# kshedden/muscato

Hardware: AMD Instinct MI355X
Metric: reads/sec (100 bp, multi-map) at 1/2/4/8 MI355X; confirm-kernel HBM GB/s vs peak (higher is better)
Workload: dtype u32

## Files before the change

muscato_amd/build.py:

```python
from __future__ import annotations

import os
import shutil
import subprocess
from concurrent.futures import ThreadPoolExecutor

HERE = os.path.dirname(os.path.abspath(__file__))
CSRC = os.path.join(HERE, "csrc")
LIB = os.path.join(HERE, "libmuscato_hip.so")
OBJ = os.path.join(HERE, "build")
SOURCES = [os.path.join(CSRC, f) for f in ("muscato_hip.hip", "match_lane_rw4.hip", "match_lane_rw8.hip", "match_lane_rw12.hip",
                                           "match_lane_rw8w.hip", "match_lane_rw12w.hip", "match_lane_rw16w.hip", "match_lane_rw8s.hip", "match_dma_rw8.hip")]
HEADERS = [os.path.join(os.path.dirname(HERE), "include", "muscato_hip.h")] + \
    [os.path.join(CSRC, f) for f in sorted(os.listdir(CSRC)) if f.endswith(".hpp")]
LANE_ONLY = os.path.join(CSRC, "kernels_match_lane.hpp")
DMA_ONLY = os.path.join(CSRC, "kernels_match_dma.hpp")
FLAGS = ["--offload-arch=gfx950", "-O3", "-std=c++17", "-fPIC", "-Wall", "-Wno-unused-function"]


def hipcc() -> str:
    for cand in (shutil.which("hipcc"), "/opt/rocm/bin/hipcc"):
        if cand and os.path.exists(cand):
            return cand
    raise RuntimeError("hipcc not found: libmuscato_hip.so cannot be built")


def needs_build() -> bool:
    if not os.path.exists(LIB):
        return True
    t = os.path.getmtime(LIB)
    return any(os.path.getmtime(p) > t for p in SOURCES + HEADERS)


HOST = os.path.join(CSRC, "host")
BIN = os.path.join(HERE, "bin")
HOST_HEADERS = [os.path.join(HOST, f) for f in sorted(os.listdir(HOST)) if f.endswith(".hpp")]
TOOLS = {"muscato": "muscato_cli.cpp", "muscato_prep_targets": "muscato_prep_targets.cpp",
         "muscato_screen": "muscato_screen.cpp", "muscato_confirm": "muscato_confirm.cpp"}
GPU_TOOLS = ("muscato", "muscato_prep_targets", "muscato_screen", "muscato_confirm")


def build_tools(force: bool = False, verbose: bool = False) -> None:
    os.makedirs(BIN, exist_ok=True)
    for name, src in TOOLS.items():
        out = os.path.join(BIN, name)
        srcp = os.path.join(HOST, src)
        deps = [srcp] + HOST_HEADERS + HEADERS
        if not force and os.path.exists(out) and all(os.path.getmtime(d) <= os.path.getmtime(out) for d in deps):
            continue
        cmd = ["g++", "-O2", "-std=c++17", "-Wall", "-pthread", "-o", out, srcp, "-lz"]
        if name in GPU_TOOLS:
            cmd += ["-L" + HERE, "-lmuscato_hip", "-Wl,-rpath,$ORIGIN/.."]
        if verbose:
            print(" ".join(cmd))
        subprocess.check_call(cmd)


CHECKS = {"read_names_plan_check": ("read_names_plan_check.cpp", ("read_names_plan.hpp",))}
SANITIZE = ["-O1", "-g", "-fsanitize=address,undefined", "-fno-sanitize-recover=all", "-static-libasan", "-static-libubsan"]


def build_checks(force: bool = False, verbose: bool = False, sanitize: bool = False, out_dir: str = BIN) -> dict:
    os.makedirs(out_dir, exist_ok=True)
    built = {}
    for name, (src, hdrs) in CHECKS.items():
        out = os.path.join(out_dir, name + ("_san" if sanitize else ""))
        srcp = os.path.join(HOST, src)
        deps = [srcp] + [os.path.join(CSRC, h) for h in hdrs]
        if force or not os.path.exists(out) or any(os.path.getmtime(d) > os.path.getmtime(out) for d in deps):
            cmd = ["g++", "-std=c++17", "-Wall"] + (SANITIZE if sanitize else ["-O2"]) + ["-o", out, srcp]
            if verbose:
                print(" ".join(cmd))
            subprocess.check_call(cmd)
        built[name] = out
    return built


def _compile(src: str, force: bool, verbose: bool, defines=(), tag: str = "") -> str:
    obj = os.path.join(OBJ, os.path.basename(src) + tag + ".o")
    base = os.path.basename(src)
    deps = [src] + [h for h in HEADERS if (h != LANE_ONLY or "match_lane" in base or "match_dma" in base) and (h != DMA_ONLY or "match_dma" in base)]
    if not force and os.path.exists(obj) and all(os.path.getmtime(d) <= os.path.getmtime(obj) for d in deps):
        return obj
    cmd = [hipcc()] + FLAGS + list(defines) + ["-c", "-o", obj, src]
    if verbose:
        print(" ".join(cmd))
    subprocess.check_call(cmd)
    return obj


def build(force: bool = False, verbose: bool = False) -> str:
    if force or needs_build():
        os.makedirs(OBJ, exist_ok=True)
        with ThreadPoolExecutor(max_workers=len(SOURCES)) as ex:
            objs = list(ex.map(lambda s: _compile(s, force, verbose), SOURCES))
        cmd = [hipcc(), "--offload-arch=gfx950", "-shared", "-fPIC", "-o", LIB] + objs + ["-ldl"]
        if verbose:
            print(" ".join(cmd))
        subprocess.check_call(cmd)
    build_tools(force=force, verbose=verbose)
    build_checks(force=force, verbose=verbose)
    return LIB


def variant(name: str, defines) -> str:
    os.makedirs(OBJ, exist_ok=True)
    out_dir = os.path.join(os.path.dirname(HERE), "build_variants")
    os.makedirs(out_dir, exist_ok=True)
    with ThreadPoolExecutor(max_workers=len(SOURCES)) as ex:
        main_defs = ["-D" + d[len("-DMAIN_"):] for d in defines if d.startswith("-DMAIN_")]
        lane_defs = [d for d in defines if not d.startswith("-DMAIN_")]
        objs = list(ex.map(lambda s: _compile(s, False, False, lane_defs if ("match_lane" in s or "match_dma" in s) else main_defs,
                                              "." + name if (("match_lane" in s or "match_dma" in s) and lane_defs) or ("match_lane" not in s and "match_dma" not in s and main_defs) else ""), SOURCES))
    out = os.path.join(out_dir, name + ".so")
    subprocess.check_call([hipcc(), "--offload-arch=gfx950", "-shared", "-fPIC", "-o", out] + objs + ["-ldl"])
    return out


if __name__ == "__main__":
    import sys
    if len(sys.argv) > 2 and sys.argv[1] == "variant":
        print(variant(sys.argv[2], sys.argv[3:]))
    else:
        print(build(force="--force" in sys.argv, verbose=True))
```

muscato_amd/csrc/muscato_hip.hip:

```cpp

#include <hip/hip_runtime.h>
#include <rccl/rccl.h>
#include <dlfcn.h>

#include <algorithm>
#include <cstdarg>
#include <cstdio>
#include <cstdlib>
#include <cstring>
#include <map>
#include <mutex>
#include <string>
#include <type_traits>
#include <vector>

#include "../../include/muscato_hip.h"

#include "ctx_state.hpp"
#include "dev_mem.hpp"
#include "index_plan.hpp"
#include "load_plan.hpp"

#include "kernels_common.hpp"
#include "kernels_index.hpp"
// ... 56 lines not shown
    }
  }
};
const Roctx& roctx() {
  static const Roctx r;
  return r;
}
struct Range {
  bool on;
  explicit Range(const char* name) : on(roctx().push != nullptr) {
    if (on) (void)roctx().push(name);
  }
  ~Range() {
    if (on) (void)roctx().pop();
  }
};

struct CaptureGuard {
  hipStream_t st = nullptr;
  bool active = false;
  hipError_t begin(hipStream_t s) {
    const hipError_t e = hipStreamBeginCapture(s, hipStreamCaptureModeThreadLocal);
    if (e == hipSuccess) {
      st = s;
      active = true;
    }
    return e;
  }
  hipError_t end(hipGraph_t* g) {
    active = false;
    return hipStreamEndCapture(st, g);
  }
  ~CaptureGuard() {
    if (!active) return;
    hipGraph_t g = nullptr;
    (void)hipStreamEndCapture(st, &g);
    if (g) (void)hipGraphDestroy(g);
    (void)hipGetLastError();
  }
};

struct TmpBufs {
  void* p[16] = {};
  int n = 0;
  template <class T>
  hipError_t alloc(T** out, size_t bytes) {
    void* q = nullptr;
    *out = nullptr;
    if (n >= 16) return hipErrorOutOfMemory;
    const hipError_t e = hipMalloc(&q, bytes ? bytes : 16);
    if (e == hipSuccess) p[n++] = q;
    *out = (T*)q;
    return e;
  }
  void release() {
    for (int i = 0; i < n; i++) (void)hipFree(p[i]);
    n = 0;
  }
  ~TmpBufs() { release(); }
};

}

using musc_load::RecShape;
using musc_load::StreamPlan;
using musc_load::stream_plan;
using musc_load::stream_plan_batch;

struct EnvKnobs : musc_index::Knobs {
  bool match_dma = false;
  bool screen_wg = false;
  int context = 0;
  bool no_x_context = false;
  bool force_wide = false;
  int debug_grid = 0;
  bool debug_sync = false;
  int graph = -1;
  bool pipeline = false;
  bool no_spec = false;
  long batch_reads = 0;
  uint64_t stage_bytes = 64ull << 20;
  uint64_t stage_lines = 1ull << 20;
  long mm_heap_lds = 0;
  void read() {
    *this = EnvKnobs();
    auto is = [](const char* v, const char* w) { return v && !strcmp(v, w); };
    const char* e = getenv("MUSC_INDEX");
    index = is(e, "classic") ? musc_index::IDX_CLASSIC : is(e, "lines") ? musc_index::IDX_LINES : is(e, "classic64") ? musc_index::IDX_CLASSIC64 : musc_index::IDX_AUTO;
    e = getenv("MUSC_MATCH");
    match_dma = is(e, "dma");
    screen_wg = is(getenv("MUSC_SCREEN"), "wg");
    e = getenv("MUSC_CONTEXT");
    context = is(e, "narrow") ? 1 : is(e, "wide") ? 2 : 0;
    no_x_context = getenv("MUSC_NO_X_CONTEXT") != nullptr;
    force_wide = getenv("MUSC_DEBUG_FORCE_WIDE") != nullptr;
    if ((e = getenv("MUSC_DEBUG_INDEX_BITS"))) index_bits = atoi(e);
    ctx_direct = (e = getenv("MUSC_DEBUG_CTX_DIRECT")) && atoi(e) > 0;
    if ((e = getenv("MUSC_DEBUG_GRID"))) debug_grid = atoi(e);
    debug_sync = getenv("MUSC_DEBUG_SYNC") != nullptr;
    if ((e = getenv("MUSC_GRAPH"))) graph = atoi(e);
    if ((e = getenv("MUSC_PIPELINE"))) pipeline = atoi(e) > 0;
    no_spec = getenv("MUSC_NO_SPEC") != nullptr;
    if ((e = getenv("MUSC_BATCH_READS"))) batch_reads = atol(e);
    if ((e = getenv("MUSC_DEBUG_INDEX_BUDGET_MB"))) index_budget_mb = atol(e);
    if ((e = getenv("MUSC_DEBUG_STAGE_BYTES")) && atoll(e) > 0) stage_bytes = (uint64_t)atoll(e);
    if ((e = getenv("MUSC_DEBUG_STAGE_LINES")) && atoll(e) > 0) stage_lines = (uint64_t)atoll(e);
    if ((e = getenv("MUSC_DEBUG_MM_HEAP_LDS"))) mm_heap_lds = atol(e);
  }
};

struct musc_ctx {
  int device = 0;
  hipStream_t stream = nullptr;
  std::string err;
  EnvKnobs env;
  musc_state::State st;

  DevPtr<uint32_t> db2;
  DevPtr<uint32_t> dbm2;
  bool db_has_x = false;
  bool reads_have_x = false;
  DevBuf<uint32_t> rdx;
  struct { uint64_t gen = 0; int wide = -1; } rdx_of;
  struct { uint64_t gen = 0; double pmatch = -1.0; int32_t mmp1 = -1; bool ok = false; } xok;
  DevPtr<uint32_t> dbx;
  uint64_t max_tlen = 0;
  struct { uint64_t gen = 0; int32_t key[CTX_MAX_W + 3] = {0}; bool ok = false; } xokdb;
  DevPtr<uint64_t> seq_off;
  uint32_t nseq = 0;
  uint64_t nbases = 0;
  uint64_t db_words = 0;
  std::vector<uint64_t> h_seq_off;

  uint64_t part_bases = 0;
  std::vector<uint32_t> part_first;
  musc_index::Kind part_kind = musc_index::K_CLASSIC64;
  uint64_t part_size = 0;
  uint32_t cur_part = 0;
  DevBuf<musc_hit> pacc;
  DevBuf<uint32_t> pbest;
  DevBuf<uint64_t> pcnt, padj;
  DevBuf<uint32_t> pflags, pflags_tmp;
  DevBuf<uint32_t> block_acc;

  musc_index::Resident idx;
  int wide = 0;
  DevMem idx_T, idx_E, ctx_T, ctx_E;
  unsigned scrt_resident = 0;
  int scrt_rw = 0;
  uint64_t idx_novf = 0;
  DevPtr<PathParams> d_pp;
  PathParams h_pp;
  bool h_pp_valid = false;
  DevPtr<MatchParams> d_mp;
  MatchParams h_mp;
  bool h_mp_valid = false;
  int spec_geom = 0;
  DevBuf<uint4> spill;

  DevPtr<uint32_t> rd;
  uint64_t rd_cap = 0;
  DevPtr<uint32_t> rdm;
  uint64_t nreads = 0;
  int rw = 0;
  uint32_t max_len = 0;
  bool reads_failed = false;

  struct Upload {
    DevPtr<uint32_t> stage;
    hipStream_t s_up = nullptr;
    std::vector<hipEvent_t> ev;
    StreamPlan plan;
    uint64_t next_piece = 0;
    uint64_t packed_upto = 0;
    uint32_t L = 0;
    bool active = false;
  } up;

  struct BatchSet {
    DevBuf<uint32_t> wb, rvalid, tbase, tcount;
    DevBuf<uint4> cdesc;
  } bs[2];
  int cur = 0;
  hipStream_t stream2 = nullptr;
  hipStream_t s_confirm = nullptr;
  hipEvent_t ev_ready[2] = {nullptr, nullptr}, ev_free[2] = {nullptr, nullptr}, ev_join = nullptr;
  DevBuf<uint32_t> scan_tmp, tcount2, tpre;
  DevBuf<uint4> stage;
  DevBuf<uint32_t> p_nx;
  DevBuf<uint16_t> nmiss_tab;
// ... 1005 lines not shown
```

muscato_amd/csrc/muscato_prep.hpp:

```cpp

#include <rocprim/device/device_radix_sort.hpp>

#define PREP_BASES_PER_WORD 21

DEV uint32_t prep_code(unsigned char ch) {
  switch (ch) {
    case 'A': return 1u;
    case 'C': return 2u;
    case 'G': return 3u;
    case 'T': return 4u;
    default: return 5u;
  }
}

MUSC_KERNEL __launch_bounds__(256) void k_prep_keys(const unsigned char* __restrict__ s,
                                                   const uint64_t* __restrict__ off,
                                                   const uint32_t* __restrict__ perm, uint64_t n, uint32_t w,
                                                   uint64_t* __restrict__ keys) {
  for (uint64_t i = (uint64_t)blockIdx.x * blockDim.x + threadIdx.x; i < n; i += (uint64_t)gridDim.x * blockDim.x) {
    const uint32_t r = perm[i];
    const uint64_t o = off[r];
    const uint64_t len = off[r + 1] - o;
    const uint64_t first = (uint64_t)w * PREP_BASES_PER_WORD;
    uint64_t key = 0;
    for (uint32_t j = 0; j < PREP_BASES_PER_WORD; j++) {
      const uint64_t q = first + j;
      if (q >= len) break;
      key |= (uint64_t)prep_code(s[o + q]) << (60 - 3 * j);
    }
    keys[i] = key;
  }
}

MUSC_KERNEL void k_prep_iota(uint32_t* __restrict__ p, uint64_t n) {
  for (uint64_t i = (uint64_t)blockIdx.x * blockDim.x + threadIdx.x; i < n; i += (uint64_t)gridDim.x * blockDim.x)
    p[i] = (uint32_t)i;
}

MUSC_KERNEL __launch_bounds__(256) void k_prep_heads(const unsigned char* __restrict__ s,
                                                    const uint64_t* __restrict__ off,
                                                    const uint32_t* __restrict__ perm, uint64_t n,
                                                    uint32_t* __restrict__ head) {
  for (uint64_t i = (uint64_t)blockIdx.x * blockDim.x + threadIdx.x; i < n; i += (uint64_t)gridDim.x * blockDim.x) {
    uint32_t h = 1;
    if (i > 0) {
      const uint32_t a = perm[i], b = perm[i - 1];
      const uint64_t oa = off[a], ob = off[b];
      const uint64_t la = off[a + 1] - oa, lb = off[b + 1] - ob;
      if (la == lb) {
        h = 0;
        for (uint64_t q = 0; q < la; q++)
          if (s[oa + q] != s[ob + q]) {
            h = 1;
            break;
          }
      }
    }
    head[i] = h;
  }
}

MUSC_KERNEL void k_prep_starts(const uint32_t* __restrict__ head, const uint32_t* __restrict__ incl, uint64_t n,
                              uint32_t* __restrict__ ustart, uint32_t* __restrict__ uhead,
                              const uint32_t* __restrict__ perm) {
  for (uint64_t i = (uint64_t)blockIdx.x * blockDim.x + threadIdx.x; i < n; i += (uint64_t)gridDim.x * blockDim.x) {
    if (head[i]) {
      ustart[incl[i] - 1] = (uint32_t)i;
      uhead[incl[i] - 1] = perm[i];
    }
    if (i == n - 1) ustart[incl[i]] = (uint32_t)n;
  }
}

MUSC_KERNEL void k_prep_pack(const unsigned char* __restrict__ s, const uint64_t* __restrict__ off,
                            const uint32_t* __restrict__ uhead, uint64_t nunique, int rw,
                            uint32_t* __restrict__ rd, uint32_t* __restrict__ rdm, uint32_t* __restrict__ has_x) {
  const uint64_t t = (uint64_t)blockIdx.x * blockDim.x + threadIdx.x;
  const uint64_t g = t / rw;
  const int j = (int)(t % rw);
  if (g >= nunique) return;
  const uint32_t r = uhead[g];
  const uint64_t o = off[r];
  const uint32_t len = (uint32_t)(off[r + 1] - o);
  if (j == rw - 1) {
    uint32_t anyx = 0;
    for (uint32_t q = 0; q < len; q++) {
      uint32_t isx;
      (void)ascii_code(s[o + q], &isx);
      anyx |= isx;
    }
    rd[t] = (len & 0xFFFFu) | (anyx ? READ_HAS_X : 0u);
    rdm[t] = 0;
    return;
  }
  uint32_t v = 0, mv = 0;
  for (int b = 0; b < 16; b++) {
    const uint32_t q = (uint32_t)j * 16 + b;
    if (q < len) {
      uint32_t isx;
      const uint32_t c = ascii_code(s[o + q], &isx);
      v |= c << (2 * b);
      mv |= isx << (2 * b);
    }
  }
  rd[t] = v;
  rdm[t] = mv;
  if (mv) atomicOr(has_x, 1u);
}

static int reads_sort_unique_dev(musc_ctx* c, const char* who, const unsigned char* d_s, const uint64_t* d_off, const uint64_t n,
                                 const Marks& m, uint32_t** order, uint32_t** ustart, uint64_t* nunique) {
  TmpBufs B;
  RecShape shape;
  uint64_t first = 0, last = 0, maxlen = 0;
  int rc = offsets_census(c, d_off, n, &first, &last, &maxlen);
  if (rc) return rc;
  if (first != 0) return fail(c, 2, "read offsets[0] must be 0");
  if ((rc = reads_shape(c, 0, maxlen, false, &shape))) return rc;

  const uint32_t nw = (uint32_t)std::max<uint64_t>((maxlen + PREP_BASES_PER_WORD - 1) / PREP_BASES_PER_WORD, 1);
  uint64_t *k0 = nullptr, *k1 = nullptr;
  uint32_t *p0 = nullptr, *p1 = nullptr;
  if ((rc = tmp_alloc(c, who, B, &k0, n * 8)) || (rc = tmp_alloc(c, who, B, &k1, n * 8)) || (rc = tmp_alloc(c, who, B, &p0, n * 4)) ||
      (rc = tmp_alloc(c, who, B, &p1, n * 4)))
    return rc;
  size_t tmp_bytes = 0;
  HIPCHK(c, rocprim::radix_sort_pairs(nullptr, tmp_bytes, k0, k1, p0, p1, (size_t)n, 0u, 63u, c->stream));
  void* tmp = nullptr;
  if ((rc = tmp_alloc(c, who, B, &tmp, tmp_bytes))) return rc;
  const dim3 grid(std::min(nblk(n, 256), MAX_GRID));
  hipLaunchKernelGGL(k_prep_iota, grid, dim3(256), 0, c->stream, p0, n);
  HIPCHK(c, hipGetLastError());
  for (uint32_t w = nw; w-- > 0;) {
    hipLaunchKernelGGL(k_prep_keys, grid, dim3(256), 0, c->stream, d_s, d_off, p0, n, w, k0);
    HIPCHK(c, hipGetLastError());
    HIPCHK(c, rocprim::radix_sort_pairs(tmp, tmp_bytes, k0, k1, p0, p1, (size_t)n, 0u, 63u, c->stream));
    std::swap(p0, p1);
  }

  uint32_t *head = nullptr, *incl = nullptr, *stmp = nullptr, *d_ustart = nullptr, *d_uhead = nullptr;
  if ((rc = tmp_alloc(c, who, B, &head, n * 4)) || (rc = tmp_alloc(c, who, B, &incl, n * 4)) ||
      (rc = tmp_alloc(c, who, B, &stmp, scan_tmp_elems(n) * 4)) || (rc = tmp_alloc(c, who, B, &d_ustart, (n + 1) * 4)) ||
      (rc = tmp_alloc(c, who, B, &d_uhead, n * 4)))
    return rc;
  hipLaunchKernelGGL(k_prep_heads, grid, dim3(256), 0, c->stream, d_s, d_off, p0, n, head);
  HIPCHK(c, hipGetLastError());
  if ((rc = scan_u32(c, head, incl, n, true, stmp))) return rc;
  hipLaunchKernelGGL(k_prep_starts, grid, dim3(256), 0, c->stream, head, incl, n, d_ustart, d_uhead, p0);
  HIPCHK(c, hipGetLastError());
  uint32_t nu32 = 0;
  HIPCHK(c, hipMemcpyAsync(&nu32, incl + (n - 1), 4, hipMemcpyDeviceToHost, c->stream));
  HIPCHK(c, hipStreamSynchronize(c->stream));
  const uint64_t nu = nu32;

  if ((rc = reads_shape(c, nu, maxlen, false, &shape)) || (rc = reads_records(c, shape, nu, maxlen, true, false))) return rc;
  const auto [rw, words] = shape;
  uint32_t* d_hasx = c->d_flag;
  HIPCHK(c, hipMemsetAsync(d_hasx, 0, 4, c->stream));
  hipLaunchKernelGGL(k_prep_pack, dim3(nblk(words, 256)), dim3(256), 0, c->stream, d_s, d_off, d_uhead, nu, rw, c->rd,
                     c->rdm, d_hasx);
  HIPCHK(c, hipGetLastError());
  HIPCHK(c, m.mark(c, 1));

  uint32_t* h_order = (uint32_t*)malloc(n * 4);
  uint32_t* h_ustart = (uint32_t*)malloc((nu + 1) * 4);
  if (!h_order || !h_ustart) {
    free(h_order);
    free(h_ustart);
    return fail(c, 7, "out of host memory for the sort order");
  }
  uint32_t hasx = 0;
  hipError_t e = hipMemcpyAsync(h_order, p0, n * 4, hipMemcpyDeviceToHost, c->stream);
  if (e == hipSuccess) e = hipMemcpyAsync(h_ustart, d_ustart, (nu + 1) * 4, hipMemcpyDeviceToHost, c->stream);
  if (e == hipSuccess) e = hipMemcpyAsync(&hasx, d_hasx, 4, hipMemcpyDeviceToHost, c->stream);
  if (e == hipSuccess) e = hipStreamSynchronize(c->stream);
  if (e != hipSuccess) {
    free(h_order);
    free(h_ustart);
    return fail(c, 10, "musc_reads_sort_unique: %s", hipGetErrorString(e));
  }
  reads_settle_x(c, hasx);
  c->stats.ms_read_prep = m.ms(0, 1);
  *order = h_order;
  *ustart = h_ustart;
  *nunique = nu;
  return 0;
}

static int reads_sort_unique_run(musc_ctx* c, const char* seqs, const uint64_t* offsets, uint64_t nreads, int on_device,
                                 uint32_t** order, uint32_t** ustart, uint64_t* nunique) {
  HIPCHK(c, hipSetDevice(c->device));
  free_reads(c);
  if (nreads >= 0xFFFFFFF0ull) return fail(c, 2, "too many reads for 32-bit read numbers");
  if (nreads == 0) {
    c->rw = 4;
    *order = (uint32_t*)malloc(4);
    *ustart = (uint32_t*)calloc(1, 4);
    if (!*order || !*ustart) return fail(c, 7, "out of host memory");
    return 0;
  }
  static const char* const who = "musc_reads_sort_unique";
  Marks m;
  int rc = m.start(c);
  if (rc) return rc;
  TmpBufs B;
  const unsigned char* d_s = nullptr;
  const uint64_t* d_off = nullptr;
  if ((rc = staged(c, who, B, (const unsigned char*)seqs, on_device ? 0 : offsets[nreads], on_device, 64, &d_s)) ||
      (rc = staged(c, who, B, offsets, (nreads + 1) * 8, on_device, 0, &d_off)))
    return rc;
  HIPCHK(c, m.mark(c, 0));
  return reads_sort_unique_dev(c, who, d_s, d_off, nreads, m, order, ustart, nunique);
}

extern "C" int musc_reads_sort_unique(musc_ctx* c, const char* seqs, const uint64_t* offsets, uint64_t nreads,
                                      int on_device, uint32_t** order, uint32_t** ustart, uint64_t* nunique) {
  if (!c) return 1;
  if (!order || !ustart || !nunique) return fail(c, 2, "musc_reads_sort_unique: NULL output pointer");
  *order = *ustart = nullptr;
  *nunique = 0;
  if ((!seqs || !offsets) && nreads) return fail(c, 2, "musc_reads_sort_unique: NULL input");
  return reads_load_done(c, reads_sort_unique_run(c, seqs, offsets, nreads, on_device, order, ustart, nunique));
}


extern "C" void musc_fastq_prep_free(musc_fastq_prep* p) {
  if (!p) return;
  free(p->name_off);
// ... 103 lines not shown
```

Measured before the change: 2.092 billion.

## Sort reads by first key word then refine only tied runs

Replaces the full LSD radix sort over every key word of every read with a sort on the first 21-base word, followed by detection of tied runs. Only the reads in tied runs are re-sorted on the remaining words and then by segment, and the result is scattered back. This avoids a radix pass over all n reads for each extra word when most prefixes are unique. The cost is extra scans, gathers and kernels, and more complex correctness, which is covered by a new host-side checker. The old path is kept behind MUSC_PREP_SORT=lsd.

Result: no change. 2.092 billion (median of 4 runs) (-0.0%).

```diff
diff --git a/muscato_amd/build.py b/muscato_amd/build.py
--- a/muscato_amd/build.py
+++ b/muscato_amd/build.py
@@ -56,7 +56,8 @@
         subprocess.check_call(cmd)
 
 
-CHECKS = {"read_names_plan_check": ("read_names_plan_check.cpp", ("read_names_plan.hpp",))}
+CHECKS = {"read_names_plan_check": ("read_names_plan_check.cpp", ("read_names_plan.hpp",)),
+          "prep_sort_plan_check": ("prep_sort_plan_check.cpp", ("prep_sort_plan.hpp",))}
 SANITIZE = ["-O1", "-g", "-fsanitize=address,undefined", "-fno-sanitize-recover=all", "-static-libasan", "-static-libubsan"]
 
 
diff --git a/muscato_amd/csrc/host/prep_sort_plan_check.cpp b/muscato_amd/csrc/host/prep_sort_plan_check.cpp
--- /dev/null
+++ b/muscato_amd/csrc/host/prep_sort_plan_check.cpp
@@ -0,0 +1,250 @@
+#include <algorithm>
+#include <cstdio>
+#include <cstdlib>
+#include <numeric>
+#include <random>
+#include <string>
+#include <vector>
+
+#include "../prep_sort_plan.hpp"
+
+using namespace musc_ps;
+
+static long g_checks = 0;
+#define CHECK(cond, ...)                                       \
+  do {                                                         \
+    g_checks++;                                                \
+    if (!(cond)) {                                             \
+      fprintf(stderr, "FAILED %s:%d: %s -- ", __FILE__, __LINE__, #cond); \
+      fprintf(stderr, __VA_ARGS__);                            \
+      fprintf(stderr, "\n");                                   \
+      exit(1);                                                 \
+    }                                                          \
+  } while (0)
+
+typedef std::vector<std::string> Reads;
+
+static int rank_of(char ch) { return ch == 'A' ? 0 : ch == 'C' ? 1 : ch == 'G' ? 2 : ch == 'T' ? 3 : 4; }
+static bool seq_less(const std::string& a, const std::string& b) {
+  const size_t k = std::min(a.size(), b.size());
+  for (size_t i = 0; i < k; i++)
+    if (rank_of(a[i]) != rank_of(b[i])) return rank_of(a[i]) < rank_of(b[i]);
+  return a.size() < b.size();
+}
+
+static uint64_t key_word(const std::string& s, uint32_t w) {
+  uint64_t key = 0;
+  for (uint32_t j = 0; j < BASES_PER_WORD; j++) {
+    const uint64_t q = (uint64_t)w * BASES_PER_WORD + j;
+    if (q >= s.size()) break;
+    key |= (uint64_t)(rank_of(s[q]) + 1) << base_shift(j);
+  }
+  return key;
+}
+static uint64_t seen(uint64_t key, BitRange r) { return (key >> r.begin) & ((1ull << (r.end - r.begin)) - 1); }
+
+struct Result {
+  std::vector<uint32_t> order, head;
+  uint32_t nw = 0;
+  uint64_t m = 0, runs = 0;
+};
+
+static Result stage(const Reads& reads) {
+  Result R;
+  const uint64_t n = reads.size();
+  uint64_t maxlen = 0;
+  for (const std::string& s : reads) maxlen = std::max<uint64_t>(maxlen, s.size());
+  const uint32_t nw = R.nw = word_count(maxlen);
+  std::vector<uint32_t> p(n);
+  std::iota(p.begin(), p.end(), 0u);
+  const BitRange b0 = word_bits(maxlen, 0);
+  std::stable_sort(p.begin(), p.end(), [&](uint32_t a, uint32_t b) { return seen(key_word(reads[a], 0), b0) < seen(key_word(reads[b], 0), b0); });
+  std::vector<uint64_t> K0(n);
+  for (uint64_t i = 0; i < n; i++) K0[i] = key_word(reads[p[i]], 0);
+  std::vector<uint32_t> h0(n), r(n), tincl(n);
+  for (uint64_t i = 0; i < n; i++) h0[i] = run_head(K0.data(), i) ? 1u : 0u;
+  uint32_t acc = 0, tacc = 0;
+  for (uint64_t i = 0; i < n; i++) {
+    r[i] = acc += h0[i];
+    tincl[i] = tacc += tied(h0.data(), n, i) ? 1u : 0u;
+  }
+  const uint64_t runs = R.runs = acc, m = R.m = tacc;
+  if (nw > 1 && m > 0) {
+    std::vector<uint32_t> pos(m), q(m), seg(m);
+    for (uint64_t i = 0; i < n; i++)
+      if (tied(h0.data(), n, i)) {
+        const uint32_t k = tincl[i] - 1;
+        pos[k] = (uint32_t)i, q[k] = p[i], seg[k] = r[i] - 1;
+      }
+    std::vector<uint32_t> slot(m);
+    std::iota(slot.begin(), slot.end(), 0u);
+    for (uint32_t w = nw; w-- > 1;) {
+      const BitRange br = word_bits(maxlen, w);
+      std::stable_sort(slot.begin(), slot.end(),
+                       [&](uint32_t a, uint32_t b) { return seen(key_word(reads[q[a]], w), br) < seen(key_word(reads[q[b]], w), br); });
+    }
+    const uint32_t sbits = seg_bits(runs);
+    if (sbits) {
+      const BitRange br{0u, sbits};
+      std::stable_sort(slot.begin(), slot.end(), [&](uint32_t a, uint32_t b) { return seen(seg[a], br) < seen(seg[b], br); });
+    }
+    for (uint64_t k = 0; k < m; k++) p[pos[k]] = q[slot[k]];
+  }
+  R.head.resize(n);
+  for (uint64_t i = 0; i < n; i++) R.head[i] = (i == 0 || h0[i] || reads[p[i]] != reads[p[i - 1]]) ? 1u : 0u;
+  R.order = p;
+  return R;
+}
+
+static Result check_case(const char* name, const Reads& reads) {
+  const Result R = stage(reads);
+  const uint64_t n = reads.size();
+  std::vector<uint32_t> exp(n);
+  std::iota(exp.begin(), exp.end(), 0u);
+  std::stable_sort(exp.begin(), exp.end(), [&](uint32_t a, uint32_t b) { return seq_less(reads[a], reads[b]); });
+  CHECK(R.order.size() == n, "%s", name);
+  for (uint64_t i = 0; i < n; i++) {
+    CHECK(R.order[i] == exp[i], "%s: position %llu holds read %u, the reference has %u", name, (unsigned long long)i, R.order[i], exp[i]);
+    const uint32_t h = (i == 0 || reads[exp[i]] != reads[exp[i - 1]]) ? 1u : 0u;
+    CHECK(R.head[i] == h, "%s: head flag of position %llu", name, (unsigned long long)i);
+  }
+  return R;
+}
+
+static std::string rnd(std::mt19937& g, size_t len, const char* alphabet, size_t na) {
+  std::string s(len, 'A');
+  for (char& ch : s) ch = alphabet[g() % na];
+  return s;
+}
+static std::string differ_at(const std::string& s, size_t at) {
+  std::string t = s;
+  t[at] = t[at] == 'G' ? 'T' : 'G';
+  return t;
+}
+
+int main() {
+  for (uint64_t L = 0; L <= 5000; L++) {
+    const uint32_t nw = word_count(L);
+    CHECK(nw >= 1 && (uint64_t)nw * BASES_PER_WORD >= L && (nw == 1 || (uint64_t)(nw - 1) * BASES_PER_WORD < L), "word count of %llu bases", (unsigned long long)L);
+    const uint32_t b = last_word_bases(L);
+    CHECK((L == 0 && b == 0) || (b >= 1 && b <= BASES_PER_WORD), "last word of %llu bases", (unsigned long long)L);
+    for (uint32_t w = 0; w < nw; w++) {
+      const BitRange r = word_bits(L, w);
+      CHECK(r.begin < r.end && r.end == KEY_END_BIT, "bits of word %u of %llu bases", w, (unsigned long long)L);
+      const std::string longest(L, 'X');
+      const uint64_t key = key_word(longest, w);
+      CHECK(seen(key, r) << r.begin == key, "word %u of %llu bases has a bit outside its range", w, (unsigned long long)L);
+      if (L) CHECK(((key >> r.begin) & 7u) != 0, "the range of word %u of %llu bases is wider than its bases", w, (unsigned long long)L);
+    }
+  }
+  for (uint32_t j = 0; j < BASES_PER_WORD; j++) CHECK(base_shift(j) == 60 - 3 * j, "shift of base %u", j);
+  CHECK(seg_bits(0) == 0 && seg_bits(1) == 0 && seg_bits(2) == 1 && seg_bits(3) == 2 && seg_bits(4) == 2 && seg_bits(5) == 3, "segment bits");
+  for (uint64_t runs = 1; runs < 70000; runs++) {
+    const uint32_t b = seg_bits(runs);
+    CHECK((runs - 1) >> b == 0 && (b == 0 || (runs - 1) >> (b - 1) == 1), "segment bits of %llu runs", (unsigned long long)runs);
+  }
+  CHECK(seg_bits(0xFFFFFFF0ull) == 32 && seg_bits(1ull << 32) == 32 && seg_bits((1ull << 32) + 1) == 33, "segment bits of large run counts");
+
+  std::mt19937 g(12345);
+  const std::string base100 = rnd(g, 100, "ACGT", 4);
+  {
+    Result R = check_case("one read", {base100});
+    CHECK(R.m == 0 && R.runs == 1, "one read");
+    R = check_case("two equal reads", {base100, base100});
+    CHECK(R.m == 2 && R.runs == 1, "two equal reads");
+    R = check_case("two unequal reads", {base100, differ_at(base100, 3)});
+    CHECK(R.m == 0 && R.runs == 2, "two unequal reads");
+  }
+  {
+    Reads v;
+    for (int i = 0; i < 500; i++) {
+      std::string s = rnd(g, 60, "ACGT", 4);
+      for (int j = 0, x = i; j < 5; j++, x /= 4) s[j] = "ACGT"[x % 4];
+      v.push_back(s);
+    }
+    const Result R = check_case("no ties", v);
+    CHECK(R.m == 0 && R.runs == 500 && R.nw == 3, "no ties");
+  }
+  {
+    const Result R = check_case("all identical", Reads(777, base100));
+    CHECK(R.m == 777 && R.runs == 1 && R.nw == 5, "all identical");
+  }
+  for (size_t L : {1u, 2u, 20u, 21u}) {
+    Reads v;
+    for (int i = 0; i < 300; i++) v.push_back(rnd(g, 1 + g() % L, "ACGTX", 5));
+    const Result R = check_case("one key word", v);
+    CHECK(R.nw == 1, "one key word");
+  }
+  for (size_t at : {21u, 41u, 42u, 62u, 63u, 83u, 84u, 99u}) {
+    Reads v = {differ_at(base100, at), base100, rnd(g, 100, "ACGT", 4), base100, differ_at(base100, at)};
+    const Result R = check_case("first difference behind word 0", v);
+    CHECK(R.m == 4 && R.nw == 5, "first difference at base %zu", at);
+  }
+  for (size_t cut : {20u, 21u, 22u, 42u, 63u}) {
+    Reads v = {base100, base100.substr(0, cut), base100.substr(0, cut + 1), rnd(g, 50, "ACGT", 4), base100.substr(0, cut)};
+    const Result R = check_case("a proper prefix", v);
+    CHECK(R.m == 4, "prefix cut at %zu", cut);
+  }
+  {
+    Reads v;
+    const std::string a(43, 'A');
+    for (int rep = 0; rep < 3; rep++)
+      for (size_t L : {1u, 20u, 21u, 22u, 42u, 43u}) v.push_back(a.substr(0, L)), v.push_back(rnd(g, L, "ACGT", 4));
+    const Result R = check_case("mixed lengths", v);
+    CHECK(R.nw == 3 && R.m > 0, "mixed lengths");
+  }
+  {
+    std::string x_in = base100, x_out = base100, x_both = base100;
+    x_in[7] = 'X', x_out[57] = 'X', x_both[20] = 'X', x_both[21] = 'X';
+    std::string t_out = base100;
+    t_out[57] = 'T';
+    const Result R = check_case("X inside and outside word 0", {x_out, x_in, base100, t_out, x_both, x_out, x_in, differ_at(base100, 57)});
+    CHECK(R.m >= 5, "X cases");
+  }
+  {
+    const std::string lo = "A" + base100.substr(1), hi = "T" + base100.substr(1), mid = "G" + base100.substr(1);
+    const Result R = check_case("stability", {hi, mid, lo, mid, hi, differ_at(mid, 50), mid, lo});
+    CHECK(R.m == 8 && R.runs == 3, "stability");
+  }
+  {
+    Reads v;
+    for (int i = 0; i < 300; i++) v.push_back(differ_at(base100, 21 + (size_t)(g() % 79)));
+    for (int i = 0; i < 200; i++) {
+      const std::string s = rnd(g, 100, "ACGT", 4);
+      v.push_back(s), v.push_back(differ_at(s, 21 + (size_t)(g() % 79)));
+    }
+    std::shuffle(v.begin(), v.end(), g);
+    const Result R = check_case("a run of 300 and runs of 2", v);
+    CHECK(R.m == 700 && R.runs == 201, "a run of 300 and runs of 2");
+  }
+  {
+    Reads v;
+    const std::string longr = rnd(g, 1000, "ACGT", 4);
+    v.push_back(longr);
+    for (int i = 0; i < 200; i++) v.push_back(i % 3 ? rnd(g, 100, "ACGT", 4) : longr.substr(0, 100));
+    v.push_back(longr.substr(0, 999));
+    const Result R = check_case("a read of 1000 bases", v);
+    CHECK(R.nw == 48 && R.m >= 60, "a read of 1000 bases");
+  }
+
+  for (uint32_t seed = 0; seed < 300; seed++) {
+    std::mt19937 h(seed);
+    const bool with_x = seed % 3 == 0;
+    static const size_t LENS[12] = {1, 5, 20, 21, 22, 42, 43, 63, 64, 100, 130, 260};
+    const size_t maxlen = LENS[seed % 12];
+    Reads pool;
+    for (int i = 0; i < 40; i++) pool.push_back(rnd(h, (seed % 5 == 0 ? 0 : 1) + h() % maxlen, with_x ? "ACGTX" : "ACGT", with_x ? 5 : 4));
+    Reads v;
+    const size_t n = 1 + h() % 600;
+    for (size_t i = 0; i < n; i++) {
+      std::string s = pool[h() % pool.size()];
+      const uint32_t u = h() % 10;
+      if (u < 2 && s.size() > 1) s.resize(1 + h() % s.size());
+      else if (u < 5 && !s.empty()) s[h() % s.size()] = "ACGTX"[h() % (with_x ? 5 : 4)];
+      v.push_back(s);
+    }
+    check_case("seeded", v);
+  }
+  printf("prep_sort_plan_check: %ld checks passed\n", g_checks);
+  return 0;
+}
diff --git a/muscato_amd/csrc/muscato_hip.hip b/muscato_amd/csrc/muscato_hip.hip
--- a/muscato_amd/csrc/muscato_hip.hip
+++ b/muscato_amd/csrc/muscato_hip.hip
@@ -162,6 +162,7 @@
   uint64_t stage_bytes = 64ull << 20;
   uint64_t stage_lines = 1ull << 20;
   long mm_heap_lds = 0;
+  bool prep_lsd = false;
   void read() {
     *this = EnvKnobs();
     auto is = [](const char* v, const char* w) { return v && !strcmp(v, w); };
@@ -186,6 +187,7 @@
     if ((e = getenv("MUSC_DEBUG_STAGE_BYTES")) && atoll(e) > 0) stage_bytes = (uint64_t)atoll(e);
     if ((e = getenv("MUSC_DEBUG_STAGE_LINES")) && atoll(e) > 0) stage_lines = (uint64_t)atoll(e);
     if ((e = getenv("MUSC_DEBUG_MM_HEAP_LDS"))) mm_heap_lds = atol(e);
+    prep_lsd = is(getenv("MUSC_PREP_SORT"), "lsd");
   }
 };
 
diff --git a/muscato_amd/csrc/muscato_prep.hpp b/muscato_amd/csrc/muscato_prep.hpp
--- a/muscato_amd/csrc/muscato_prep.hpp
+++ b/muscato_amd/csrc/muscato_prep.hpp
@@ -1,7 +1,10 @@
 
 #include <rocprim/device/device_radix_sort.hpp>
 
+#include "prep_sort_plan.hpp"
+
 #define PREP_BASES_PER_WORD 21
+static_assert(PREP_BASES_PER_WORD == musc_ps::BASES_PER_WORD, "one key layout");
 
 DEV uint32_t prep_code(unsigned char ch) {
   switch (ch) {
@@ -13,23 +16,68 @@
   }
 }
 
+DEV uint64_t prep_key_word(const unsigned char* __restrict__ s, const uint64_t* __restrict__ off, uint32_t r, uint32_t w) {
+  const uint64_t o = off[r];
+  const uint64_t len = off[r + 1] - o;
+  const uint64_t first = (uint64_t)w * PREP_BASES_PER_WORD;
+  uint64_t key = 0;
+  for (uint32_t j = 0; j < PREP_BASES_PER_WORD; j++) {
+    const uint64_t q = first + j;
+    if (q >= len) break;
+    key |= (uint64_t)prep_code(s[o + q]) << musc_ps::base_shift(j);
+  }
+  return key;
+}
+
 MUSC_KERNEL __launch_bounds__(256) void k_prep_keys(const unsigned char* __restrict__ s,
                                                    const uint64_t* __restrict__ off,
                                                    const uint32_t* __restrict__ perm, uint64_t n, uint32_t w,
                                                    uint64_t* __restrict__ keys) {
+  for (uint64_t i = (uint64_t)blockIdx.x * blockDim.x + threadIdx.x; i < n; i += (uint64_t)gridDim.x * blockDim.x)
+    keys[i] = prep_key_word(s, off, perm[i], w);
+}
+
+MUSC_KERNEL __launch_bounds__(256) void k_prep_keys_slot(const unsigned char* __restrict__ s,
+                                                        const uint64_t* __restrict__ off,
+                                                        const uint32_t* __restrict__ q,
+                                                        const uint32_t* __restrict__ slot, uint64_t m, uint32_t w,
+                                                        uint64_t* __restrict__ keys) {
+  for (uint64_t j = (uint64_t)blockIdx.x * blockDim.x + threadIdx.x; j < m; j += (uint64_t)gridDim.x * blockDim.x)
+    keys[j] = prep_key_word(s, off, q[slot[j]], w);
+}
+
+MUSC_KERNEL void k_prep_runs(const uint64_t* __restrict__ k0, uint64_t n, uint32_t* __restrict__ h0) {
+  for (uint64_t i = (uint64_t)blockIdx.x * blockDim.x + threadIdx.x; i < n; i += (uint64_t)gridDim.x * blockDim.x)
+    h0[i] = musc_ps::run_head(k0, i) ? 1u : 0u;
+}
+
+MUSC_KERNEL void k_prep_tied(const uint32_t* __restrict__ h0, uint64_t n, uint32_t* __restrict__ t) {
+  for (uint64_t i = (uint64_t)blockIdx.x * blockDim.x + threadIdx.x; i < n; i += (uint64_t)gridDim.x * blockDim.x)
+    t[i] = musc_ps::tied(h0, n, i) ? 1u : 0u;
+}
+
+MUSC_KERNEL void k_prep_tied_gather(const uint32_t* __restrict__ h0, const uint32_t* __restrict__ rincl,
+                                   const uint32_t* __restrict__ tincl, const uint32_t* __restrict__ p, uint64_t n,
+                                   uint32_t* __restrict__ pos, uint32_t* __restrict__ q, uint32_t* __restrict__ seg) {
   for (uint64_t i = (uint64_t)blockIdx.x * blockDim.x + threadIdx.x; i < n; i += (uint64_t)gridDim.x * blockDim.x) {
-    const uint32_t r = perm[i];
-    const uint64_t o = off[r];
-    const uint64_t len = off[r + 1] - o;
-    const uint64_t first = (uint64_t)w * PREP_BASES_PER_WORD;
-    uint64_t key = 0;
-    for (uint32_t j = 0; j < PREP_BASES_PER_WORD; j++) {
-      const uint64_t q = first + j;
-      if (q >= len) break;
-      key |= (uint64_t)prep_code(s[o + q]) << (60 - 3 * j);
-    }
-    keys[i] = key;
-  }
+    if (!musc_ps::tied(h0, n, i)) continue;
+    const uint32_t k = tincl[i] - 1;
+    pos[k] = (uint32_t)i;
+    q[k] = p[i];
+    seg[k] = rincl[i] - 1;
+  }
+}
+
+MUSC_KERNEL void k_prep_seg_keys(const uint32_t* __restrict__ seg, const uint32_t* __restrict__ slot, uint64_t m,
+                                uint32_t* __restrict__ keys) {
+  for (uint64_t j = (uint64_t)blockIdx.x * blockDim.x + threadIdx.x; j < m; j += (uint64_t)gridDim.x * blockDim.x)
+    keys[j] = seg[slot[j]];
+}
+
+MUSC_KERNEL void k_prep_put_back(const uint32_t* __restrict__ pos, const uint32_t* __restrict__ q,
+                                const uint32_t* __restrict__ slot, uint64_t m, uint32_t* __restrict__ p) {
+  for (uint64_t k = (uint64_t)blockIdx.x * blockDim.x + threadIdx.x; k < m; k += (uint64_t)gridDim.x * blockDim.x)
+    p[pos[k]] = q[slot[k]];
 }
 
 MUSC_KERNEL void k_prep_iota(uint32_t* __restrict__ p, uint64_t n) {
@@ -39,11 +87,11 @@
 
 MUSC_KERNEL __launch_bounds__(256) void k_prep_heads(const unsigned char* __restrict__ s,
                                                     const uint64_t* __restrict__ off,
-                                                    const uint32_t* __restrict__ perm, uint64_t n,
-                                                    uint32_t* __restrict__ head) {
+                                                    const uint32_t* __restrict__ perm, uint64_t n, const uint32_t* h0,
+                                                    uint32_t* head) {
   for (uint64_t i = (uint64_t)blockIdx.x * blockDim.x + threadIdx.x; i < n; i += (uint64_t)gridDim.x * blockDim.x) {
     uint32_t h = 1;
-    if (i > 0) {
+    if (i > 0 && !(h0 && h0[i])) {
       const uint32_t a = perm[i], b = perm[i - 1];
       const uint64_t oa = off[a], ob = off[b];
       const uint64_t la = off[a + 1] - oa, lb = off[b + 1] - ob;
@@ -108,6 +156,113 @@
   if (mv) atomicOr(has_x, 1u);
 }
 
+struct PrepBufs {
+  uint64_t *k0 = nullptr, *k1 = nullptr;
+  uint32_t *p0 = nullptr, *p1 = nullptr;
+  uint32_t *head = nullptr, *incl = nullptr, *stmp = nullptr, *d_ustart = nullptr, *d_uhead = nullptr;
+  void* tmp = nullptr;
+  size_t tmp_bytes = 0;
+};
+
+static int reads_sort_lsd(musc_ctx* c, const char* who, TmpBufs& B, PrepBufs& P, const unsigned char* d_s, const uint64_t* d_off,
+                          const uint64_t n, const uint32_t nw, uint32_t** ord) {
+  int rc = 0;
+  uint64_t *k0 = P.k0, *k1 = P.k1;
+  uint32_t *p0 = P.p0, *p1 = P.p1;
+  HIPCHK(c, rocprim::radix_sort_pairs(nullptr, P.tmp_bytes, k0, k1, p0, p1, (size_t)n, 0u, 63u, c->stream));
+  if ((rc = tmp_alloc(c, who, B, &P.tmp, P.tmp_bytes))) return rc;
+  const dim3 grid(std::min(nblk(n, 256), MAX_GRID));
+  hipLaunchKernelGGL(k_prep_iota, grid, dim3(256), 0, c->stream, p0, n);
+  HIPCHK(c, hipGetLastError());
+  for (uint32_t w = nw; w-- > 0;) {
+    hipLaunchKernelGGL(k_prep_keys, grid, dim3(256), 0, c->stream, d_s, d_off, p0, n, w, k0);
+    HIPCHK(c, hipGetLastError());
+    HIPCHK(c, rocprim::radix_sort_pairs(P.tmp, P.tmp_bytes, k0, k1, p0, p1, (size_t)n, 0u, 63u, c->stream));
+    std::swap(p0, p1);
+  }
+  *ord = p0;
+  return 0;
+}
+
+static int reads_sort_tied(musc_ctx* c, const char* who, TmpBufs& B, PrepBufs& P, const unsigned char* d_s, const uint64_t* d_off,
+                           const uint64_t n, const uint64_t maxlen, const uint32_t nw, uint32_t** ord, const uint32_t** h0) {
+  namespace ps = musc_ps;
+  int rc = 0;
+  const ps::BitRange b0 = ps::word_bits(maxlen, 0);
+  HIPCHK(c, rocprim::radix_sort_pairs(nullptr, P.tmp_bytes, P.k0, P.k1, P.p0, P.p1, (size_t)n, b0.begin, b0.end, c->stream));
+  if ((rc = tmp_alloc(c, who, B, &P.tmp, P.tmp_bytes))) return rc;
+  const dim3 grid(std::min(nblk(n, 256), MAX_GRID));
+  hipLaunchKernelGGL(k_prep_iota, grid, dim3(256), 0, c->stream, P.p0, n);
+  HIPCHK(c, hipGetLastError());
+  hipLaunchKernelGGL(k_prep_keys, grid, dim3(256), 0, c->stream, d_s, d_off, P.p0, n, 0u, P.k0);
+  HIPCHK(c, hipGetLastError());
+  HIPCHK(c, rocprim::radix_sort_pairs(P.tmp, P.tmp_bytes, P.k0, P.k1, P.p0, P.p1, (size_t)n, b0.begin, b0.end, c->stream));
+  uint32_t* const p = P.p1;
+  *ord = p;
+  uint32_t *const hd = P.head, *const rincl = P.incl, *const tincl = P.p0;
+  *h0 = hd;
+  hipLaunchKernelGGL(k_prep_runs, grid, dim3(256), 0, c->stream, P.k1, n, hd);
+  HIPCHK(c, hipGetLastError());
+  if (nw == 1) return 0;
+  if ((rc = scan_u32(c, hd, rincl, n, true, P.stmp))) return rc;
+  hipLaunchKernelGGL(k_prep_tied, grid, dim3(256), 0, c->stream, hd, n, tincl);
+  HIPCHK(c, hipGetLastError());
+  if ((rc = scan_u32(c, tincl, tincl, n, true, P.stmp))) return rc;
+  uint32_t back[2] = {0, 0};
+  HIPCHK(c, hipMemcpyAsync(&back[0], rincl + (n - 1), 4, hipMemcpyDeviceToHost, c->stream));
+  HIPCHK(c, hipMemcpyAsync(&back[1], tincl + (n - 1), 4, hipMemcpyDeviceToHost, c->stream));
+  HIPCHK(c, hipStreamSynchronize(c->stream));
+  const uint64_t runs = back[0], m = back[1];
+  if (m == 0) return 0;
+  if (m > n || runs == 0 || runs > n)
+    return fail(c, 11, "%s: %llu tied reads in %llu runs of %llu reads", who, (unsigned long long)m, (unsigned long long)runs,
+                (unsigned long long)n);
+  uint32_t *const pos = P.d_ustart, *const q = P.d_uhead, *seg = nullptr;
+  if ((rc = tmp_alloc(c, who, B, &seg, m * 4))) return rc;
+  hipLaunchKernelGGL(k_prep_tied_gather, grid, dim3(256), 0, c->stream, hd, rincl, tincl, p, n, pos, q, seg);
+  HIPCHK(c, hipGetLastError());
+  uint64_t *ka = P.k0, *kb = P.k1;
+  uint32_t *sa = P.p0, *sb = P.incl;
+  const uint32_t sbits = ps::seg_bits(runs);
+  size_t need = 0;
+  for (uint32_t w = nw; w-- > 1;) {
+    const ps::BitRange br = ps::word_bits(maxlen, w);
+    size_t t = 0;
+    HIPCHK(c, rocprim::radix_sort_pairs(nullptr, t, ka, kb, sa, sb, (size_t)m, br.begin, br.end, c->stream));
+    need = std::max(need, t);
+  }
+  if (sbits) {
+    size_t t = 0;
+    HIPCHK(c, rocprim::radix_sort_pairs(nullptr, t, (uint32_t*)ka, (uint32_t*)kb, sa, sb, (size_t)m, 0u, sbits, c->stream));
+    need = std::max(need, t);
+  }
+  if (need > P.tmp_bytes) {
+    if ((rc = tmp_alloc(c, who, B, &P.tmp, need))) return rc;
+    P.tmp_bytes = need;
+  }
+  const dim3 mgrid(std::min(nblk(m, 256), MAX_GRID));
+  hipLaunchKernelGGL(k_prep_iota, mgrid, dim3(256), 0, c->stream, sa, m);
+  HIPCHK(c, hipGetLastError());
+  for (uint32_t w = nw; w-- > 1;) {
+    const ps::BitRange br = ps::word_bits(maxlen, w);
+    size_t t = P.tmp_bytes;
+    hipLaunchKernelGGL(k_prep_keys_slot, mgrid, dim3(256), 0, c->stream, d_s, d_off, q, sa, m, w, ka);
+    HIPCHK(c, hipGetLastError());
+    HIPCHK(c, rocprim::radix_sort_pairs(P.tmp, t, ka, kb, sa, sb, (size_t)m, br.begin, br.end, c->stream));
+    std::swap(sa, sb);
+  }
+  if (sbits) {
+    size_t t = P.tmp_bytes;
+    hipLaunchKernelGGL(k_prep_seg_keys, mgrid, dim3(256), 0, c->stream, seg, sa, m, (uint32_t*)ka);
+    HIPCHK(c, hipGetLastError());
+    HIPCHK(c, rocprim::radix_sort_pairs(P.tmp, t, (uint32_t*)ka, (uint32_t*)kb, sa, sb, (size_t)m, 0u, sbits, c->stream));
+    std::swap(sa, sb);
+  }
+  hipLaunchKernelGGL(k_prep_put_back, mgrid, dim3(256), 0, c->stream, pos, q, sa, m, p);
+  HIPCHK(c, hipGetLastError());
+  return 0;
+}
+
 static int reads_sort_unique_dev(musc_ctx* c, const char* who, const unsigned char* d_s, const uint64_t* d_off, const uint64_t n,
                                  const Marks& m, uint32_t** order, uint32_t** ustart, uint64_t* nunique) {
   TmpBufs B;
@@ -118,32 +273,21 @@
   if (first != 0) return fail(c, 2, "read offsets[0] must be 0");
   if ((rc = reads_shape(c, 0, maxlen, false, &shape))) return rc;
 
-  const uint32_t nw = (uint32_t)std::max<uint64_t>((maxlen + PREP_BASES_PER_WORD - 1) / PREP_BASES_PER_WORD, 1);
-  uint64_t *k0 = nullptr, *k1 = nullptr;
-  uint32_t *p0 = nullptr, *p1 = nullptr;
-  if ((rc = tmp_alloc(c, who, B, &k0, n * 8)) || (rc = tmp_alloc(c, who, B, &k1, n * 8)) || (rc = tmp_alloc(c, who, B, &p0, n * 4)) ||
-      (rc = tmp_alloc(c, who, B, &p1, n * 4)))
+  const uint32_t nw = musc_ps::word_count(maxlen);
+  PrepBufs P;
+  if ((rc = tmp_alloc(c, who, B, &P.k0, n * 8)) || (rc = tmp_alloc(c, who, B, &P.k1, n * 8)) || (rc = tmp_alloc(c, who, B, &P.p0, n * 4)) ||
+      (rc = tmp_alloc(c, who, B, &P.p1, n * 4)) || (rc = tmp_alloc(c, who, B, &P.head, n * 4)) || (rc = tmp_alloc(c, who, B, &P.incl, n * 4)) ||
+      (rc = tmp_alloc(c, who, B, &P.stmp, scan_tmp_elems(n) * 4)) || (rc = tmp_alloc(c, who, B, &P.d_ustart, (n + 1) * 4)) ||
+      (rc = tmp_alloc(c, who, B, &P.d_uhead, n * 4)))
     return rc;
-  size_t tmp_bytes = 0;
-  HIPCHK(c, rocprim::radix_sort_pairs(nullptr, tmp_bytes, k0, k1, p0, p1, (size_t)n, 0u, 63u, c->stream));
-  void* tmp = nullptr;
-  if ((rc = tmp_alloc(c, who, B, &tmp, tmp_bytes))) return rc;
+  uint32_t* p0 = nullptr;
+  const uint32_t* h0 = nullptr;
+  if ((rc = c->env.prep_lsd ? reads_sort_lsd(c, who, B, P, d_s, d_off, n, nw, &p0) : reads_sort_tied(c, who, B, P, d_s, d_off, n, maxlen, nw, &p0, &h0)))
+    return rc;
+
+  uint32_t *const head = P.head, *const incl = P.incl, *const stmp = P.stmp, *const d_ustart = P.d_ustart, *const d_uhead = P.d_uhead;
   const dim3 grid(std::min(nblk(n, 256), MAX_GRID));
-  hipLaunchKernelGGL(k_prep_iota, grid, dim3(256), 0, c->stream, p0, n);
-  HIPCHK(c, hipGetLastError());
-  for (uint32_t w = nw; w-- > 0;) {
-    hipLaunchKernelGGL(k_prep_keys, grid, dim3(256), 0, c->stream, d_s, d_off, p0, n, w, k0);
-    HIPCHK(c, hipGetLastError());
-    HIPCHK(c, rocprim::radix_sort_pairs(tmp, tmp_bytes, k0, k1, p0, p1, (size_t)n, 0u, 63u, c->stream));
-    std::swap(p0, p1);
-  }
-
-  uint32_t *head = nullptr, *incl = nullptr, *stmp = nullptr, *d_ustart = nullptr, *d_uhead = nullptr;
-  if ((rc = tmp_alloc(c, who, B, &head, n * 4)) || (rc = tmp_alloc(c, who, B, &incl, n * 4)) ||
-      (rc = tmp_alloc(c, who, B, &stmp, scan_tmp_elems(n) * 4)) || (rc = tmp_alloc(c, who, B, &d_ustart, (n + 1) * 4)) ||
-      (rc = tmp_alloc(c, who, B, &d_uhead, n * 4)))
-    return rc;
-  hipLaunchKernelGGL(k_prep_heads, grid, dim3(256), 0, c->stream, d_s, d_off, p0, n, head);
+  hipLaunchKernelGGL(k_prep_heads, grid, dim3(256), 0, c->stream, d_s, d_off, p0, n, h0, head);
   HIPCHK(c, hipGetLastError());
   if ((rc = scan_u32(c, head, incl, n, true, stmp))) return rc;
   hipLaunchKernelGGL(k_prep_starts, grid, dim3(256), 0, c->stream, head, incl, n, d_ustart, d_uhead, p0);
diff --git a/muscato_amd/csrc/prep_sort_plan.hpp b/muscato_amd/csrc/prep_sort_plan.hpp
--- /dev/null
+++ b/muscato_amd/csrc/prep_sort_plan.hpp
@@ -0,0 +1,45 @@
+#pragma once
+
+#include <cstdint>
+
+#if defined(__HIPCC__)
+#define PS_HD __host__ __device__ inline
+#else
+#define PS_HD inline
+#endif
+
+namespace musc_ps {
+
+constexpr uint32_t BASES_PER_WORD = 21, BITS_PER_BASE = 3;
+constexpr uint32_t KEY_END_BIT = BASES_PER_WORD * BITS_PER_BASE;
+
+PS_HD uint32_t word_count(uint64_t maxlen) {
+  const uint64_t nw = (maxlen + BASES_PER_WORD - 1) / BASES_PER_WORD;
+  return nw ? (uint32_t)nw : 1u;
+}
+
+PS_HD uint32_t last_word_bases(uint64_t maxlen) { return (uint32_t)(maxlen - (uint64_t)BASES_PER_WORD * (word_count(maxlen) - 1)); }
+
+PS_HD uint32_t base_shift(uint32_t j) { return KEY_END_BIT - BITS_PER_BASE * (j + 1); }
+
+struct BitRange {
+  uint32_t begin, end;
+};
+
+PS_HD BitRange word_bits(uint64_t maxlen, uint32_t w) {
+  if (w + 1 < word_count(maxlen)) return BitRange{0u, KEY_END_BIT};
+  const uint32_t b = last_word_bases(maxlen);
+  return BitRange{KEY_END_BIT - BITS_PER_BASE * (b ? b : 1u), KEY_END_BIT};
+}
+
+PS_HD uint32_t seg_bits(uint64_t runs) {
+  uint32_t b = 0;
+  for (uint64_t v = runs ? runs - 1 : 0; v; v >>= 1) b++;
+  return b;
+}
+
+PS_HD bool run_head(const uint64_t* k0, uint64_t i) { return i == 0 || k0[i] != k0[i - 1]; }
+
+PS_HD bool tied(const uint32_t* h0, uint64_t n, uint64_t i) { return !h0[i] || (i + 1 < n && !h0[i + 1]); }
+
+}
diff --git a/profiles/read_prep.py b/profiles/read_prep.py
--- /dev/null
+++ b/profiles/read_prep.py
@@ -0,0 +1,173 @@
+#!/usr/bin/env python3
+import csv
+import glob
+import json
+import os
+import statistics
+import sys
+
+ROOT = os.path.dirname(os.path.dirname(os.path.abspath(__file__)))
+OUT = os.path.join(ROOT, "profiles", "read_prep.jsonl")
+sys.path.insert(0, ROOT)
+
+
+def emit(rec, keep=True):
+    if keep:
+        with open(OUT, "a") as f:
+            f.write(json.dumps(rec) + "\n")
+    print(json.dumps(rec), flush=True)
+
+
+def raw_reads(key):
+    import torch
+    from muscato_amd import synth
+    wl = synth.workload_for(key, 1)
+    device = torch.device("cuda", 0)
+    seed = synth.SEED_BASE + sum(ord(c) for c in wl.seed_key)
+    targets = synth.gen_targets(wl, device, seed)
+    U = wl.n_unique_reads
+    reads = synth.sort_reads(synth.gen_unique_reads(wl, targets, device, seed + 7919))
+    del targets
+    g = torch.Generator(device=device)
+    g.manual_seed(seed + 17)
+    n = wl.n_raw_reads
+    extra = torch.randint(0, U, (n - U,), device=device, generator=g)
+    raw = torch.cat([reads, reads[extra]])[torch.randperm(n, device=device, generator=g)]
+    del extra, reads
+    off = synth.offsets_for(n, wl.read_len, device)
+    torch.cuda.synchronize()
+    return raw, off, n
+
+
+def timed(eng, raw, off, n, reps):
+    ms, nu = [], 0
+    for _ in range(reps + 1):
+        order, ustart = eng.sort_unique_reads_arrays(raw.data_ptr(), off.data_ptr(), n, True)
+        ms.append(round(eng.stats()["ms_read_prep"], 3))
+        nu = len(ustart) - 1
+    return ms[1:], nu
+
+
+def run(reps, key):
+    from muscato_amd import Engine
+    raw, off, n = raw_reads(key)
+    with Engine(0) as eng:
+        ms, nu = timed(eng, raw, off, n, reps)
+    emit({"run": True, "workload": key, "lib": os.environ.get("MUSC_LIB_PATH", "tree"), "sort": os.environ.get("MUSC_PREP_SORT", "default"),
+          "raw_reads": n, "distinct": nu, "read_prep_device_ms": ms, "median_ms": statistics.median(ms)}, keep=False)
+
+
+def stats(d, tag):
+    paths = glob.glob(os.path.join(d, "**", "*kernel_stats.csv"), recursive=True)
+    if len(paths) != 1:
+        raise SystemExit("expected one kernel_stats.csv under %s, found %d" % (d, len(paths)))
+    with open(paths[0]) as f:
+        rows = list(csv.DictReader(f))
+    total = sum(float(r["TotalDurationNs"]) for r in rows)
+    dst = os.path.join(ROOT, "profiles", "read_prep_kernel_stats_%s.csv" % tag)
+    with open(dst, "w", newline="") as f:
+        w = csv.writer(f)
+        w.writerow(["Name", "Calls", "TotalDurationNs", "AverageNs", "Percentage"])
+        for r in sorted(rows, key=lambda r: -float(r["TotalDurationNs"])):
+            t = float(r["TotalDurationNs"])
+            if t / total >= 0.001:
+                w.writerow([r["Name"][:160], r["Calls"], int(t), int(float(r["AverageNs"])), "%.2f" % (100 * t / total)])
+    print(dst)
+
+
+def census(key):
+    import torch
+    raw, off, n = raw_reads(key)
+    lut = torch.full((256,), 5, dtype=torch.int64, device=raw.device)
+    for ch, code in zip(b"ACGT", (1, 2, 3, 4)):
+        lut[ch] = code
+    key0 = torch.zeros(n, dtype=torch.int64, device=raw.device)
+    for j in range(min(21, raw.shape[1])):
+        key0 |= lut[raw[:, j].long()] << (60 - 3 * j)
+    _, counts = torch.unique(key0, return_counts=True)
+    m = int(counts[counts >= 2].sum())
+    emit({"census": True, "workload": key, "n": n, "runs": int(counts.numel()), "tied_runs": int((counts >= 2).sum()), "m": m,
+          "m_over_n": m / n, "longest_run": int(counts.max())})
+
+
+def tied3(nd, reps):
+    import torch
+    from muscato_amd import Engine
+    device = torch.device("cuda", 0)
+    g = torch.Generator(device=device)
+    g.manual_seed(3)
+    lut = torch.tensor(list(b"ACGT"), dtype=torch.uint8, device=device)
+    one = lut[torch.randint(0, 4, (nd, 100), device=device, generator=g)]
+    raw = one.repeat(3, 1)[torch.randperm(3 * nd, device=device, generator=g)].contiguous()
+    off = torch.arange(3 * nd + 1, dtype=torch.int64, device=device) * 100
+    torch.cuda.synchronize()
+    rec = {"tied3": True, "lib": os.environ.get("MUSC_LIB_PATH", "tree"), "reads": 3 * nd, "key_words": 5}
+    with Engine(0) as eng:
+        for path in ("default", "lsd", "default", "lsd"):
+            if path == "lsd":
+                os.environ["MUSC_PREP_SORT"] = "lsd"
+            else:
+                os.environ.pop("MUSC_PREP_SORT", None)
+            eng.reload_env()
+            ms, nu = timed(eng, raw, off, 3 * nd, reps)
+            rec.setdefault(path + "_ms", []).extend(ms)
+            rec["distinct"] = nu
+    os.environ.pop("MUSC_PREP_SORT", None)
+    rec["default_median_ms"], rec["lsd_median_ms"] = statistics.median(rec["default_ms"]), statistics.median(rec["lsd_ms"])
+    rec["default_over_lsd"] = rec["default_median_ms"] / rec["lsd_median_ms"]
+    emit(rec)
+
+
+def bench(tag, path):
+    line = [ln for ln in open(path).read().splitlines() if ln.startswith("{")][-1]
+    j = json.loads(line)
+    rec = {"bench": True, "tag": tag, "read_prep_device_ms": j["one_off"]["read_prep_device_ms"], "distinct": j["one_off"]["distinct"],
+           "index_build_ms": j["one_off"]["index_build_ms"], "value": j["value"], "unit": j.get("unit")}
+    if "equals_torch_sort" in j["one_off"]:
+        rec["equals_torch_sort"] = j["one_off"]["equals_torch_sort"]
+    for k in ("kernel_pipeline", "ms_per_step"):
+        if k in j:
+            rec[k] = j[k]
+    emit(rec)
+
+
+def verdict():
+    recs = [json.loads(ln) for ln in open(OUT) if ln.strip()]
+    by = {}
+    for r in recs:
+        if r.get("bench") and "equals_torch_sort" not in r:
+            by.setdefault(r["tag"], []).append(r["read_prep_device_ms"])
+    out = {"verdict": True}
+    for tag, v in by.items():
+        out[tag] = {"runs": len(v), "median_ms": statistics.median(v), "spread_ms": max(v) - min(v)}
+    if "parent" in by and "new" in by:
+        diff = out["parent"]["median_ms"] - out["new"]["median_ms"]
+        out["difference_ms"] = diff
+        out["new_over_parent"] = out["new"]["median_ms"] / out["parent"]["median_ms"]
+        out["exceeds_five_parent_spreads"] = abs(diff) > 5 * out["parent"]["spread_ms"]
+    emit(out)
+
+
+def main():
+    a = sys.argv[1:]
+    if not a:
+        raise SystemExit(__doc__)
+    if a[0] == "run":
+        run(int(a[1]) if len(a) > 1 else 5, a[2] if len(a) > 2 else "cfg3")
+    elif a[0] == "stats":
+        stats(a[1], a[2])
+    elif a[0] == "census":
+        census(a[1] if len(a) > 1 else "cfg3")
+    elif a[0] == "tied3":
+        tied3(int(a[1]) if len(a) > 1 else 10_000_000, int(a[2]) if len(a) > 2 else 3)
+    elif a[0] == "bench":
+        bench(a[1], a[2])
+    elif a[0] == "verdict":
+        verdict()
+    else:
+        raise SystemExit(__doc__)
+    return 0
+
+
+if __name__ == "__main__":
+    sys.exit(main())
```
